# JJanai/slowflow

Measured on AMD Instinct MI355X. Metric: Mpix*solver-iters/s at 1024x436 (whole coarse-to-fine path), higher is better.
Workload: dtype f32

## Files before the change

slowflow_amd/csrc/job.hip:

```cpp
#include <algorithm>
#include <cmath>
#include <cstring>
#include <memory>
#include <vector>

#include "sfa_internal.h"

#pragma clang fp contract(off)

namespace sfa {

enum { P_WX = 0, P_WY, P_UU, P_VV, P_DU, P_DV, P_ODU, P_ODV, P_SH, P_SV, P_A11, P_A12, P_A22, P_B1, P_B2, P_OCC, P_DPSIS, P_COUNT };
struct Level {
    int w = 0, h = 0, pitch = 0, lstride = 0, ref = 0, F = 0, nb = 0;
    bool fused = true;
    long pl = 0, es = 0;
    long off_masks = 0, off_warp = 0, off_stacks = 0, off_tmp = 0;
    float *base = nullptr;
    float *pbase = nullptr;
    float *plane(int i) const { return i < 2 ? pbase + (long)i * pl : base + (long)(i - 2) * pl; }
    float *mask(int s) const { return base + off_masks + (long)s * pl; }
    float *stack(int s, int toref) const { return base + off_stacks + ((long)s * 2 + toref) * 24 * pl; }
    float *warp(int s, int sp1) const { return base + off_warp + (long)(s + sp1) * 3 * pl; }
    float *frame(int f) const { return pbase + 2 * pl + (long)f * 3 * pl; }
    float *tmp() const { return base + off_tmp; }
    Geo geo() const { return Geo{w, h, pitch, pl, es, nb, WMask::first(nb), nullptr}; }
    Geo geo(const WMask &active) const { return Geo{w, h, pitch, pl, es, nb, active, nullptr}; }
    static long persistent_floats(int pitch, int h, int ref) { return (long)pitch * h * (2 + (2L * ref + 1) * 3); }
    static long transient_floats(int pitch, int h, int ref, bool fused) {
        return (long)pitch * h * ((P_COUNT - 2) + 2 * ref + (2L * ref + 1) * 3 + (fused ? 0 : 2L * ref * 2 * 24));
    }
    void layout(float *transient, float *persistent, int w_, int h_, int lstride_, int ref_, int nb_, long es_, bool fused_) {
        base = transient; pbase = persistent; w = w_; h = h_; pitch = dev_pitch(w_); lstride = lstride_; ref = ref_; F = 2 * ref_ + 1; nb = nb_; es = es_; fused = fused_;
        pl = (long)pitch * h;
        off_masks = (long)(P_COUNT - 2) * pl;
        off_warp = off_masks + 2L * ref * pl;
        off_stacks = off_warp + (2L * ref + 1) * 3 * pl;
        off_tmp = off_warp;
    }
};
struct ChannelWeights { const float *dev = nullptr; long pl = 0, es = 0; int pitch = 0, stride0 = 0; };

static const float *pair_image(const Level &L, int s, int sp1) { return (s + sp1 - L.ref == 0) ? L.frame(s + sp1) : L.warp(s, sp1); }

static bool get_derivatives(sfa_ctx *c, const Level &L, const sfa_params &p, const Geo &g, const bool need_toref[2 * SFA_MAX_REF], bool with_smoothness = false) {
    const int ref = L.ref;
    WarpJobs J;
    J.n = 0;
    for (int f = p.one_direction ? ref + 1 : 0; f <= 2 * ref; f++) {
        if (f == ref) continue;
        const int s = f < ref ? f : f - 1;
        J.job[J.n++] = WarpJob{L.frame(f) - L.base, L.warp(f < ref ? f : f - 1, f < ref ? 0 : 1) - L.base, L.mask(s) - L.base, f - ref};
    }
    const bool smoothed = with_smoothness && L.fused &&
                          launch_warp_smooth(c, g, J, L.base, L.plane(P_WX), L.plane(P_WY), p.smoothing, L.plane(P_SH), L.plane(P_SV), L.plane(P_DPSIS), p.alpha, pen(p.robust_reg));
    if (!smoothed) launch_warp_jobs(c, g, J, L.base, L.plane(P_WX), L.plane(P_WY));
    for (int s = p.one_direction ? ref : 0; s < 2 * ref; s++) {
        if (L.fused) continue;
        const float *w_s = pair_image(L, s, 0), *w_sp1 = pair_image(L, s, 1);
        launch_deriv_stack(c, g, L.stack(s, 0), w_s, w_sp1, L.es, L.es);
        if (need_toref[s]) {
            if (s < ref) launch_deriv_stack(c, g, L.stack(s, 1), w_s, L.frame(ref), L.es, L.es);
            else         launch_deriv_stack(c, g, L.stack(s, 1), L.frame(ref), w_sp1, L.es, L.es);
        }
    }
    return smoothed;
}

static int optimize_occlusions(sfa_ctx *c, const Level &L, const sfa_params &p, const Geo &g, DevMem &scratch) {
    const int ref = L.ref;
    const size_t n = (size_t)L.nb * L.pl;
    SFA_TRY(scratch.alloc(c, (2 + kCutWorkPlanes) * n * sizeof(float)));
    float *d0 = scratch.f(), *d1 = d0 + n, *work = d1 + n;
    OccArgs oa;
    memset(&oa, 0, sizeof oa);
    oa.nslots = 2 * ref; oa.hd = p.delta / 3.0f; oa.hg = p.gamma / 3.0f; oa.penalty = p.occlusion_penalty;
    oa.color = pen(p.robust_color); oa.grad = pen(p.robust_grad);
    for (int s = 0; s < 2 * ref; s++) {
        const float *i1 = pair_image(L, s, 0), *i2 = pair_image(L, s, 1);
        const float *r1 = s < ref ? i1 : L.frame(ref), *r2 = s < ref ? L.frame(ref) : i2;
        const int idx = std::max(ref - s - 1, s - ref);
        oa.slot[s] = OccSlot{i1 - L.base, i2 - L.base, r1 - L.base, r2 - L.base, L.off_masks + (long)s * L.pl, p.rho[idx], p.omega[idx], s >= ref ? 0 : 1};
    }
    launch_occ_costs(c, g, oa, L.base, d0, d1, L.pl);
    return run_grid_cut(c, g, L.plane(P_OCC), L.es, d0, d1, work, p.occlusion_alpha);
}


static Term data_term(const Level &L, const sfa_params &p, int slot, int is_ref, float weight, float s) {
    const float *i1 = pair_image(L, slot, 0), *i2 = pair_image(L, slot, 1);
    if (is_ref) { if (slot < L.ref) i2 = L.frame(L.ref); else i1 = L.frame(L.ref); }
    return Term{L.off_stacks + ((long)slot * 2 + is_ref) * 24 * L.pl, L.off_masks + (long)slot * L.pl, weight * (p.delta / 3.0f), weight * (p.gamma / 3.0f), s, is_ref,
                i1 - L.base, i2 - L.base, slot < L.ref};
}
static int data_terms(sfa_ctx *c, const Level &L, const sfa_params &p, const ChannelWeights &cw, AssembleArgs &aa, bool need_toref[2 * SFA_MAX_REF]) {
    const int ref = L.ref;
    memset(&aa, 0, sizeof aa);
    for (int s = 0; s < ref; s++) {
        const int a = ref - 1 - s;
        if (!p.one_direction) {
            if (p.rho[a] > 0) aa.t[aa.n++] = data_term(L, p, s, 0, p.rho[a], (float)(s - ref));
            if (p.omega[a] > 0) { aa.t[aa.n++] = data_term(L, p, s, 1, p.omega[a], (float)(s - ref)); need_toref[s] = true; }
        }
        if (p.rho[s] > 0) aa.t[aa.n++] = data_term(L, p, ref + s, 0, p.rho[s], (float)s);
        if (p.omega[s] > 0) { aa.t[aa.n++] = data_term(L, p, ref + s, 1, p.omega[s], (float)(s + 1)); need_toref[ref + s] = true; }
        aa.data_norm += p.rho[s] + p.omega[s];
    }
    for (int t = 0; t < aa.n; t++)
        if (aa.t[t].is_ref && aa.t[t].s == 0) return set_error(c, SFA_ERR_REF_FRAME, "Frame compared to reference frame is the reference frame itself!");
    aa.one_direction = p.one_direction; aa.dt_norm = p.dataterm_norm;
    aa.color = pen(p.robust_color); aa.grad = pen(p.robust_grad);
    aa.chw = cw.dev; aa.chw_pl = cw.pl; aa.chw_es = cw.es; aa.chw_pitch = cw.pitch; aa.chw_stride0 = cw.stride0; aa.lstride = L.lstride;
    aa.accumulate = 0; aa.do_laplacian = 1;
    return SFA_OK;
}

struct LevelPlan {
// ... 584 lines not shown
```

slowflow_amd/csrc/kernels.hip:

```cpp
#include "sfa_device.h"
#include "sor_device.h"

#pragma clang fp contract(off)

namespace sfa {

__device__ __forceinline__ float psi_vec(const PenaltyDev &p, float xsq) {
    const float e2 = p.eps * p.eps;
    switch (p.id) {
    case 0: return 1.0f;
    case 2: return __fdiv_rn(1.0f, 2.0f * e2 + xsq);
    case 3: {
        float out = __fdiv_rn(1.0f, 2.0f * sqrt_rn(xsq + e2));
        if (sqrt_rn(xsq) > p.trunc) out = 0.0f;
        return out;
    }
    case 4: {
        float t = e2 + xsq;
        t = t * t;
        return __fdiv_rn(e2 + 2.0f * xsq, t);
    }
    default: return __fdiv_rn(1.0f, 2.0f * sqrt_rn(xsq + e2));
    }
}
// ... 11 lines not shown
        t = t * t;
        return (float)((e2d + (double)(2.0f * xsq)) / (double)t);
    }
    default: return (float)(1.0 / (2.0 * __dsqrt_rn((double)xsq + e2d)));
    }
}

__global__ void k_warp(float *__restrict__ dst3, float *__restrict__ mask, const float *__restrict__ src3, const float *__restrict__ wx,
                       const float *__restrict__ wy, Geo g, int factor, long src_es) {
    const int b = blockIdx.z;
    if (!elem_active(g, b)) return;
    const int x = blockIdx.x * BX + threadIdx.x, y = blockIdx.y * BY + threadIdx.y;
    if (x >= g.w || y >= g.h) return;
    dst3 += b * g.es; wx += b * g.es; wy += b * g.es; src3 += b * src_es;
    const size_t o = (size_t)y * g.pitch + x;
    if (factor == 0) {
        for (int k = 0; k < 3; k++) dst3[k * g.pl + o] = src3[k * g.pl + o];
        return;
    }
    const float xx = x + factor * wx[o];
    const float yy = y + factor * wy[o];
    const int xi = floor_to_int_x86(xx), yi = floor_to_int_x86(yy);
    const float dx = xx - xi, dy = yy - yi;
    if (mask) mask[b * g.es + o] = (xx >= 0 && xx <= g.w - 1 && yy >= 0 && yy <= g.h - 1) ? 1.0f : 0.0f;
    const int x1 = clampi(xi, 0, g.w - 1), x2 = clampi(xi + 1, 0, g.w - 1);
    const int y1 = clampi(yi, 0, g.h - 1), y2 = clampi(yi + 1, 0, g.h - 1);
    const float ax = 1.0f - dx, ay = 1.0f - dy;
    for (int k = 0; k < 3; k++) {
        const float *s = src3 + k * g.pl;
        dst3[k * g.pl + o] = s[(size_t)y1 * g.pitch + x1] * ax * ay + s[(size_t)y1 * g.pitch + x2] * dx * ay
                           + s[(size_t)y2 * g.pitch + x1] * ax * dy + s[(size_t)y2 * g.pitch + x2] * dx * dy;
    }
}
template <bool ALLJ>
__global__ void k_warp_jobs(WarpJobs J, float *__restrict__ base, const float *__restrict__ wx, const float *__restrict__ wy, Geo g) {
    const int b = ALLJ ? blockIdx.z : blockIdx.z / J.n, j0 = ALLJ ? 0 : blockIdx.z % J.n;
    if (!elem_active(g, b)) return;
    const int x = blockIdx.x * BX + threadIdx.x, y = blockIdx.y * BY + threadIdx.y;
    if (x >= g.w || y >= g.h) return;
    const long eb = b * g.es;
    const size_t o = (size_t)y * g.pitch + x;
    const float fx0 = wx[eb + o], fy0 = wy[eb + o];
    for (int j = j0; j <= (ALLJ ? J.n - 1 : j0); j++) {
        const int factor = J.job[j].factor;
        const float *src3 = base + eb + J.job[j].src_off;
        float *dst3 = base + eb + J.job[j].dst_off;
        const float xx = x + factor * fx0;
        const float yy = y + factor * fy0;
        const int xi = floor_to_int_x86(xx), yi = floor_to_int_x86(yy);
        const float dx = xx - xi, dy = yy - yi;
        if (J.job[j].mask_off >= 0) base[eb + J.job[j].mask_off + o] = (xx >= 0 && xx <= g.w - 1 && yy >= 0 && yy <= g.h - 1) ? 1.0f : 0.0f;
        const int x1 = clampi(xi, 0, g.w - 1), x2 = clampi(xi + 1, 0, g.w - 1);
        const int y1 = clampi(yi, 0, g.h - 1), y2 = clampi(yi + 1, 0, g.h - 1);
        const float ax = 1.0f - dx, ay = 1.0f - dy;
        float out[3];
#pragma unroll
        for (int k = 0; k < 3; k++) {
            const float *s = src3 + k * g.pl;
            out[k] = s[(size_t)y1 * g.pitch + x1] * ax * ay + s[(size_t)y1 * g.pitch + x2] * dx * ay
                   + s[(size_t)y2 * g.pitch + x1] * ax * dy + s[(size_t)y2 * g.pitch + x2] * dx * dy;
        }
#pragma unroll
        for (int k = 0; k < 3; k++) dst3[k * g.pl + o] = out[k];
    }
}
void launch_warp_jobs(sfa_ctx *c, const Geo &g, const WarpJobs &J, float *base, const float *wx, const float *wy) {
    if (J.n <= 0) return;
    const bool allj = sw_int(Switches::WARP_ALLJ, 1) != 0;
    if (allj) hipLaunchKernelGGL(k_warp_jobs<true>, grid2d(g), block2d(), 0, c->stream, J, base, wx, wy, g);
    else hipLaunchKernelGGL(k_warp_jobs<false>, grid2d(g, J.n), block2d(), 0, c->stream, J, base, wx, wy, g);
}
void launch_warp(sfa_ctx *c, const Geo &g, float *dst3, float *mask, const float *src3, const float *wx, const float *wy, int factor, long src_es) {
    hipLaunchKernelGGL(k_warp, grid2d(g), block2d(), 0, c->stream, dst3, mask, src3, wx, wy, g, factor, src_es);
}


constexpr int DT_X = 64, DT_Y = 16, DT_H = 4, DT_W = DT_X + 2 * DT_H, DT_R = DT_Y + 2 * DT_H;
struct TileAcc {
    const float *t; int x0, y0;
    __device__ __forceinline__ float operator()(int x, int y) const { return t[(y - y0) * DT_W + (x - x0)]; }
};
__global__ void __launch_bounds__(256) k_deriv_stack(float *__restrict__ out24, const float *__restrict__ I1, const float *__restrict__ I2, Geo g, long es1, long es2) {
    __shared__ float sM[DT_R * DT_W], sZ[DT_R * DT_W], sX[DT_R * DT_W], sY[DT_R * DT_W];
    const int b = blockIdx.z / 3, ch = blockIdx.z % 3;
    if (!elem_active(g, b)) return;
    const int x0 = blockIdx.x * DT_X - DT_H, y0 = blockIdx.y * DT_Y - DT_H;
    const float *a = I1 + b * es1 + ch * g.pl, *bb = I2 + b * es2 + ch * g.pl;
    for (int i = threadIdx.x; i < DT_R * DT_W; i += 256) {
        const int x = x0 + i % DT_W, y = y0 + i / DT_W;
        if (x >= 0 && x < g.w && y >= 0 && y < g.h) {
            const size_t o = (size_t)y * g.pitch + x;
            const float va = a[o], vb = bb[o];
            sM[i] = 0.5f * (vb + va);
            sZ[i] = va - vb;
        }
    }
    __syncthreads();
    const TileAcc m{sM, x0, y0};
    constexpr int W1 = DT_X + 4, R1 = DT_Y + 4;
    for (int i = threadIdx.x; i < R1 * W1; i += 256) {
        const int lx = 2 + i % W1, ly = 2 + i / W1;
        const int x = x0 + lx, y = y0 + ly;
        if (x >= 0 && x < g.w && y >= 0 && y < g.h) {
// ... 280 lines not shown
#endif
    auto ld = [](const float *ubase, unsigned boff) { return *reinterpret_cast<const float *>(reinterpret_cast<const char *>(ubase) + boff); };
    auto st = [](float *ubase, unsigned boff, float v) {
        if (SFA_X_WS & 32) __builtin_nontemporal_store(v, reinterpret_cast<float *>(reinterpret_cast<char *>(ubase) + boff));
        else *reinterpret_cast<float *>(reinterpret_cast<char *>(ubase) + boff) = v;
    };
    const unsigned pitch4 = 4u * (unsigned)g.pitch;
    const float *pu = uu_ + eb, *pv = vv_ + eb, *pd = dps_ + eb;
    for (int i = tid; i < SM_R * SM_W; i += 64 * WS_ROWS) {
        const int gx = x0 + i % SM_W, gy = y0 + i / SM_W;
        if (gx >= 0 && gx < g.w && gy >= 0 && gy < g.h) {
            const unsigned o4 = (unsigned)gy * pitch4 + 4u * (unsigned)gx;
            tU[i] = ld(pu, o4); tV[i] = ld(pv, o4); tD[i] = ld(pd, o4);
        }
    }
    __syncthreads();
    const SmTile uu{tU, x0, y0}, vv{tV, x0, y0}, dps{tD, x0, y0};
    const int w = g.w, h = g.h;
    const int x = x0 + 1 + threadIdx.x;
    sh += eb; sv += eb;
    for (int k = 0; k < SM_Y / WS_ROWS; k++) {
        const int y = y0 + 1 + threadIdx.y + WS_ROWS * k;
        if (x >= g.pitch || y >= h) continue;
        const unsigned o4 = (unsigned)y * pitch4 + 4u * (unsigned)x;
        if (x >= w) { st(sh, o4, 0.0f); st(sv, o4, 0.0f); continue; }
        const float fx0 = uu(x, y), fy0 = vv(x, y);
        auto gather = [&](int j, float(&out)[3]) {
            const int factor = J.job[j].factor;
            const float *src3 = base + eb + J.job[j].src_off;
            const float xx = x + factor * fx0;
            const float yy = y + factor * fy0;
            const int xi = floor_to_int_x86(xx), yi = floor_to_int_x86(yy);
            const float dx = xx - xi, dy = yy - yi;
            if (J.job[j].mask_off >= 0) st(base + eb + J.job[j].mask_off, o4, (xx >= 0 && xx <= g.w - 1 && yy >= 0 && yy <= g.h - 1) ? 1.0f : 0.0f);
            const int x1 = clampi(xi, 0, g.w - 1), x2 = clampi(xi + 1, 0, g.w - 1);
            const int y1 = clampi(yi, 0, g.h - 1), y2 = clampi(yi + 1, 0, g.h - 1);
            const float ax = 1.0f - dx, ay = 1.0f - dy;
            const unsigned r1 = (unsigned)y1 * pitch4, r2 = (unsigned)y2 * pitch4, c1 = 4u * (unsigned)x1, c2 = 4u * (unsigned)x2;
            const unsigned o11 = (SFA_X_WS & 1) ? o4 : r1 + c1, o12 = (SFA_X_WS & 1) ? o4 : r1 + c2, o21 = (SFA_X_WS & 1) ? o4 : r2 + c1, o22 = (SFA_X_WS & 1) ? o4 : r2 + c2;
#pragma unroll
            for (int ch = 0; ch < 3; ch++) {
                const float *sp = src3 + ch * g.pl;
                if (SFA_X_WS & 8) { out[ch] = ax * ay + dx * dy; continue; }
#if defined(SFA_WS_LDNT) && SFA_WS_LDNT
                auto ldn = [](const float *ubase, unsigned boff) { return __builtin_nontemporal_load(reinterpret_cast<const float *>(reinterpret_cast<const char *>(ubase) + boff)); };
                out[ch] = ldn(sp, o11) * ax * ay + ldn(sp, o12) * dx * ay + ldn(sp, o21) * ax * dy + ldn(sp, o22) * dx * dy;
#else
                out[ch] = ld(sp, o11) * ax * ay + ld(sp, o12) * dx * ay + ld(sp, o21) * ax * dy + ld(sp, o22) * dx * dy;
#endif
            }
        };
        auto put = [&](int j, const float(&out)[3]) {
            float *dst3 = base + eb + J.job[j].dst_off;
#pragma unroll
            for (int ch = 0; ch < 3; ch++) {
                if (SFA_X_WS & 4) continue;
                if (SFA_WS_NT) __builtin_nontemporal_store(out[ch], reinterpret_cast<float *>(reinterpret_cast<char *>(dst3 + ch * g.pl) + o4));
                else st(dst3 + ch * g.pl, o4, out[ch]);
            }
        };
        float out0[3] = {0, 0, 0}, out1[3] = {0, 0, 0};
        gather(0, out0);
        if (J.n > 1) gather(1, out1);
        float outh = 0.0f, outv = 0.0f;
        if (x < w - 1) {
            const float ux1 = uu(x + 1, y) - uu(x, y), vx1 = vv(x + 1, y) - vv(x, y);
            float t = 0.0f, t2 = 0.0f;
// ... 2 lines not shown
                t2 = 0.5f * (d3y(vv, x, y, h) + d3y(vv, x + 1, y, h));
            }
            t = ux1 * ux1 + t * t;
            t2 = vx1 * vx1 + t2 * t2;
            t = t + t2;
            outh = (dps(x, y) + dps(x + 1, y)) * alpha * ((SFA_X_WS & 2) ? t : psi_scalar(reg, t));
        }
        if (y < h - 1) {
            const float uy1 = uu(x, y + 1) - uu(x, y), vy1 = vv(x, y + 1) - vv(x, y);
            float t = 0.0f, t2 = 0.0f;
            if (method == 1) {
                t = 0.5f * (d3x(uu, x, y, w) + d3x(uu, x, y + 1, w));
                t2 = 0.5f * (d3x(vv, x, y, w) + d3x(vv, x, y + 1, w));
            }
            t = uy1 * uy1 + t * t;
            t2 = vy1 * vy1 + t2 * t2;
            t = t + t2;
            outv = (dps(x, y) + dps(x, y + 1)) * alpha * ((SFA_X_WS & 2) ? t : psi_scalar(reg, t));
        }
        st(sh, o4, outh);
        st(sv, o4, outv);
        put(0, out0);
        if (J.n > 1) put(1, out1);
        for (int j = 2; j < J.n; j++) {
            float o3[3];
            gather(j, o3);
            put(j, o3);
        }
    }
}
bool launch_warp_smooth(sfa_ctx *c, const Geo &g, const WarpJobs &J, float *base, const float *wx, const float *wy, int method, float *sh, float *sv,
                        const float *dpsis, float alpha, PenaltyDev reg) {
    const bool off = sw_given(Switches::NO_WARP_SMOOTH);
    if (off || method > 1 || J.n <= 0) return false;
    if ((unsigned long long)g.pl * 4ull >= (1ull << 32)) return false;
#if defined(SFA_WS_XCD) && SFA_WS_XCD
    const unsigned tiles = (unsigned)((g.pitch + SM_X - 1) / SM_X) * (unsigned)((g.h + SM_Y - 1) / SM_Y) * (unsigned)g.nb;
    hipLaunchKernelGGL(k_warp_smooth, dim3((tiles + 7) / 8 * 8), dim3(64, WS_ROWS), 0, c->stream, J, base, method, sh, sv, wx, wy, dpsis, g, alpha, reg);
#else
    hipLaunchKernelGGL(k_warp_smooth, dim3((g.pitch + SM_X - 1) / SM_X, (g.h + SM_Y - 1) / SM_Y, g.nb), dim3(64, WS_ROWS), 0, c->stream, J, base, method, sh, sv, wx, wy,
                       dpsis, g, alpha, reg);
#endif
    return true;
}

template <class SrcAcc>
__device__ __forceinline__ float laplacian_gather(float bval, const SrcAcc &src, const SrcAcc &wh, const SrcAcc &wv, int x, int y, int w, int h) {
    const float c = src(x, y);
    if (x > 0) bval -= wh(x - 1, y) * (c - src(x - 1, y));
    if (x < w - 1) bval += wh(x, y) * (src(x + 1, y) - c);
    if (y > 0) bval -= wv(x, y - 1) * (c - src(x, y - 1));
    if (y < h - 1) bval += wv(x, y) * (src(x, y + 1) - c);
    return bval;
}
__global__ void k_sub_laplacian(float *__restrict__ dst, const float *__restrict__ src, const float *__restrict__ wh, const float *__restrict__ wv, Geo g) {
    const int b = blockIdx.z;
    const int x = blockIdx.x * BX + threadIdx.x, y = blockIdx.y * BY + threadIdx.y;
    if (x >= g.w || y >= g.h) return;
    PlaneAcc s{src + b * g.es, g.pitch}, h_{wh + b * g.es, g.pitch}, v_{wv + b * g.es, g.pitch};
    const size_t o = b * g.es + (size_t)y * g.pitch + x;
    dst[o] = laplacian_gather(dst[o], s, h_, v_, x, y, g.w, g.h);
}
void launch_sub_laplacian(sfa_ctx *c, const Geo &g, float *dst, const float *src, const float *wh, const float *wv) {
    hipLaunchKernelGGL(k_sub_laplacian, grid2d(g), block2d(), 0, c->stream, dst, src, wh, wv, g);
}

#define EPS2F (0.001f * 0.001f)
// ... 838 lines not shown
    const int dt_norm = FAST ? 1 : a.dt_norm;
    PenaltyDev pcolor = a.color, pgrad = a.grad;
    if (FAST) { pcolor.id = FAST; pgrad.id = FAST; }
    Acc A[NP];
    float u[NP], v[NP], wk[NP][3], fwd[NP], bwd[NP], oc[NP];
    bool ok[NP];
#pragma unroll
    for (int k = 0; k < NP; k++) {
        const int y = y0 + DT_H + ty + NR * k;
        ok[k] = x < g.w && y < g.h;
        A[k].a11 = A[k].a12 = A[k].a22 = A[k].b1 = A[k].b2 = 0.0f;
        u[k] = v[k] = 0.0f; fwd[k] = bwd[k] = 0.0f; oc[k] = 0.0f;
        wk[k][0] = wk[k][1] = wk[k][2] = 1.0f;
        if (!ok[k]) continue;
        const size_t o = (size_t)y * g.pitch + x;
        if (!ZUV) { u[k] = du[eb + o]; v[k] = dv[eb + o]; }
        if (!FAST && a.chw) channel_weights(a, b, x, y, wk[k]);
        if (!(SFA_X_AI & 128)) oc[k] = occ[eb + o];
    }
    const bool need_g = a.do_laplacian || a.op.sa;
    auto stage_epilogue_operands = [&]() {
        if (!need_g) return;
        for (int i0 = 0; i0 < K::NGQ; i0 += NT) {
            const int item = i0 + (int)threadIdx.x;
            const int q = item % K::QM, row = (item / K::QM) % K::GR, pl = item / (K::QM * K::GR);
            const int gy = y0 + DT_H - 1 + row, gx = x0 + 4 * q;
            const float *src = pl == 0 ? uu : pl == 1 ? vv : pl == 2 ? sh : sv;
            if (!(SFA_X_AI & 32) && item < K::NGQ && gy >= 0 && gy < g.h && gx >= 0 && gx + 3 < g.pitch && (pl >= 2 || a.do_laplacian))
                dma16(src + eb + (size_t)gy * g.pitch + gx, lds_addr(lds + 4 * (i0 + 64 * ty)));
        }
    };
    AT_MARK(13);
    if (a.n == 0) stage_epilogue_operands();
    float mk[NP];
    for (int t = 0; t < a.n; t++) {
        const Term &T = a.t[t];
        AT_MARK(0);
        if (t > 0) __syncthreads();
        AT_MARK(1);
        SFA_PRIO(SFA_PRIO_STAGE);
        asm_issue_image_dma<K>(base + eb + T.i1_off, base + eb + T.i2_off, g, x0, y0, tx, ty);
#pragma unroll
        for (int k = 0; k < NP; k++) {
            const size_t o = (size_t)(y0 + DT_H + ty + NR * k) * g.pitch + x;
            mk[k] = ok[k] && !(SFA_X_AI & 128) ? base[eb + T.mask_off + o] : 0.0f;
        }
        AT_MARK(2);
        asm volatile("s_waitcnt vmcnt(0)" ::: "memory");
#pragma unroll
        for (int k = 0; k < NP; k++) {
            asm volatile("" : "+v"(mk[k]), "+v"(oc[k]));
            if (!FAST) asm volatile("" : "+v"(wk[k][0]), "+v"(wk[k][1]), "+v"(wk[k][2]));
            if (!ZUV) asm volatile("" : "+v"(u[k]), "+v"(v[k]));
        }
        AT_MARK(3);
        __syncthreads();
        AT_MARK(4);
        if (t == 0) {
#pragma unroll
            for (int k = 0; k < NP; k++) mask_weights(oc[k], a.data_norm, fwd[k], bwd[k]);
        }
        if (tile_in) asm_convert<K, true>(base + eb + T.i1_off, base + eb + T.i2_off, g, x0, y0);
        else asm_convert<K, false>(base + eb + T.i1_off, base + eb + T.i2_off, g, x0, y0);
        AT_MARK(5);
        AT_MARK(0);
        __syncthreads();
        AT_MARK(6);
        SFA_PRIO(SFA_PRIO_STAGE);
        if (tile_in) asm_stage1<K, true>(g, x0, y0);
        else asm_stage1<K, false>(g, x0, y0);
        AT_MARK(7);
        __syncthreads();
        AT_MARK(8);
        SFA_PRIO(0);
        if (t == a.n - 1) stage_epilogue_operands();
#pragma unroll
        for (int k = 0; k < NP; k++) {
            const int yl = ty + NR * k, y = y0 + DT_H + yl;
            if (y >= g.h) break;
            Px p = asm_pixel_derivatives<K>(g, x0, y0, tx, yl, y);
#pragma unroll
            for (int ch = 0; ch < 3; ch++) p.wk[ch] = FAST ? 1.0f : wk[k][ch];
            if (!ok[k]) continue;
            float m = mk[k];
            if (!a.one_direction || !T.backward) m = T.backward ? 1.0f * bwd[k] * m : 1.0f * fwd[k] * m;
            if (SFA_X_AI & 16) {
                for (int ch = 0; ch < 3; ch++) {
                    A[k].a11 += p.ix[ch] + p.ixx[ch] + m; A[k].a12 += p.iy[ch] + p.ixy[ch]; A[k].a22 += p.iz[ch] + p.iyy[ch]; A[k].b1 += p.ixz[ch]; A[k].b2 += p.iyz[ch];
                }
            } else if (T.is_ref) term_ref<ZUV, FAST != 0>(A[k], p, m, u[k], v[k], T.hd, T.hg, T.s, dt_norm, pcolor, pgrad, a.chain_ok != 0);
            else          term_succ<ZUV, FAST != 0>(A[k], p, m, u[k], v[k], T.hd, T.hg, T.s, dt_norm, pcolor, pgrad, a.chain_ok != 0);
        }
    }
    AT_MARK(0);
    if (need_g) {
        asm volatile("s_waitcnt vmcnt(0)" ::: "memory");
        __syncthreads();
    }
    AT_MARK(9);
    SFA_PRIO(SFA_PRIO_STAGE);
#pragma unroll
    for (int k = 0; k < NP; k++) {
        if (!ok[k]) continue;
        const int yl = ty + NR * k, y = y0 + DT_H + yl;
        asm_epilogue_pixel<K>(a, g, A[k], u[k], v[k], x0, y0, tx, yl, x, y);
        if (!a.op.sa) {
            const size_t o = eb + (size_t)y * g.pitch + x;
            a11[o] = A[k].a11; a12[o] = A[k].a12; a22[o] = A[k].a22; b1[o] = A[k].b1; b2[o] = A[k].b2;
        }
    }
    if (!a.op.sa) return;
    AT_MARK(10);
    __syncthreads();
    AT_MARK(11);
    asm_store_operand_tile<K>(a.op, g, b, x0 + DT_H, y0 + DT_H);
#ifdef SFA_ASM_TIMING
    AT_MARK(12);
// ... 788 lines not shown
```

slowflow_amd/csrc/occlusion.hip:

```cpp
#include "sfa_device.h"
#include <vector>

#include <cstdlib>
#include <utility>

#pragma clang fp contract(off)

namespace sfa {

__device__ __forceinline__ float psi_apply_vec(const PenaltyDev &p, float xsq) {
    const float e2 = p.eps * p.eps;
    switch (p.id) {
    case 0: return xsq;
    case 2: return (float)log(1 + 0.5 * (double)xsq / (double)e2);
    case 3: {
        float out = sqrt_rn(xsq + e2);
        if (sqrt_rn(xsq) > p.trunc) out = sqrt_rn(p.trunc + e2);
        return out;
    }
    case 4: return __fdiv_rn(xsq, (xsq + 1.0f) * (xsq + 1.0f));
    default: return sqrt_rn(xsq + e2);
    }
}

#define DT_SCALE_GRAPHC 0.01f

constexpr int OC_X = 64, OC_Y = 8, OC_W = OC_X + 4, OC_R = OC_Y + 4, OC_NT = 512;
struct OccTileAcc {
    const float *t; int x0, y0;
    __device__ __forceinline__ float operator()(int x, int y) const { return t[(y - y0) * OC_W + (x - x0)]; }
};

__global__ void __launch_bounds__(OC_NT) k_occ_costs(OccArgs a, const float *__restrict__ base, float *__restrict__ d0, float *__restrict__ d1, long des, Geo g) {
    __shared__ float sZ[3][OC_R * OC_W];
    const int b = blockIdx.z;
    if (!elem_active(g, b)) return;
    const long eb = b * g.es;
    const int x0 = blockIdx.x * OC_X - 2, y0 = blockIdx.y * OC_Y - 2;
    const int tx = threadIdx.x & 63;
    const int ty = __builtin_amdgcn_readfirstlane(threadIdx.x >> 6);
    const int x = x0 + 2 + tx, y = y0 + 2 + ty;
    const bool ok = x < g.w && y < g.h;
    const bool y_in = y >= 2 && y + 2 < g.h;
    const int c = (ty + 2) * OC_W + (tx + 2);
    float e[2] = {0.0f, 0.0f}, n[2] = {0.0f, 0.0f};
    for (int s = 0; s < a.nslots; s++) {
        const OccSlot &S = a.slot[s];
        const float m = ok ? base[eb + S.mask_off + (size_t)y * g.pitch + x] : 0.0f;
        float term = 0.0f;
        for (int kind = 0; kind < 2; kind++) {
            const float wgt = kind ? S.omega : S.rho;
            if (wgt == 0.0f && kind == 1) continue;
            const float *pa = base + eb + (kind ? S.r1_off : S.s1_off), *pb = base + eb + (kind ? S.r2_off : S.s2_off);
            __syncthreads();
            constexpr int OC_Q = (OC_W + 2 + 3) / 4;
            for (int i = threadIdx.x; i < 3 * OC_R * OC_Q; i += OC_NT) {
                const int ch = i / (OC_R * OC_Q), r = (i / OC_Q) % OC_R, qa = i % OC_Q;
                const int gy = y0 + r, gx = x0 - 2 + 4 * qa;
                if (gy < 0 || gy >= g.h) continue;
                const size_t ro = ch * g.pl + (size_t)gy * g.pitch;
                float z[4];
                if (gx >= 0 && gx + 3 < g.w) {
                    const float4 va = *reinterpret_cast<const float4 *>(pa + ro + gx), vb = *reinterpret_cast<const float4 *>(pb + ro + gx);
                    z[0] = va.x - vb.x; z[1] = va.y - vb.y; z[2] = va.z - vb.z; z[3] = va.w - vb.w;
                } else {
#pragma unroll
                    for (int e = 0; e < 4; e++) { const int cx = clampi(gx + e, 0, g.w - 1); z[e] = pa[ro + cx] - pb[ro + cx]; }
                }
#pragma unroll
                for (int e = 0; e < 4; e++) {
                    const int q = 4 * qa - 2 + e;
                    if (q >= 0 && q < OC_W) sZ[ch][r * OC_W + q] = z[e];
                }
            }
            __syncthreads();
            if (!ok) continue;
            float iz[3], ixz[3], iyz[3];
#pragma unroll
            for (int ch = 0; ch < 3; ch++) {
                const float *Z = sZ[ch];
                iz[ch] = Z[c];
                ixz[ch] = tap5(Z[c - 2], Z[c - 1], Z[c], Z[c + 1], Z[c + 2]);
                if (y_in) iyz[ch] = tap5(Z[c - 2 * OC_W], Z[c - OC_W], Z[c], Z[c + OC_W], Z[c + 2 * OC_W]);
                else      iyz[ch] = d5y(OccTileAcc{Z, x0, y0}, x, y, g.h);
            }
            const float pc = psi_apply_vec(a.color, iz[0] * iz[0] + iz[1] * iz[1] + iz[2] * iz[2]);
            const float pg = psi_apply_vec(a.grad, ixz[0] * ixz[0] + ixz[1] * ixz[1] + ixz[2] * ixz[2] + iyz[0] * iyz[0] + iyz[1] * iyz[1] + iyz[2] * iyz[2]);
            if (kind == 0) term = wgt * a.hd * m * pc;
            else           term += wgt * a.hd * m * pc;
            term += wgt * a.hg * m * pg;
        }
        const int l = S.label;
        e[l] += term;
        n[l] += m * (S.rho + S.rho + S.omega + S.omega);
    }
    if (!ok) return;
    const size_t o = b * des + (size_t)y * g.pitch + x;
#pragma unroll
    for (int l = 0; l < 2; l++) {
        if (n[l] == 0) n[l] = 1;
        const float cst = __fdiv_rn(DT_SCALE_GRAPHC * e[l], n[l]) + a.penalty * l;
        (l ? d1 : d0)[o] = cst;
    }
}
void launch_occ_costs(sfa_ctx *c, const Geo &g, const OccArgs &a, const float *base, float *d0, float *d1, long des) {
    hipLaunchKernelGGL(k_occ_costs, dim3((g.w + OC_X - 1) / OC_X, (g.h + OC_Y - 1) / OC_Y, g.nb), dim3(OC_NT), 0, c->stream, a, base, d0, d1, des, g);
}

constexpr int kCutInf = 1 << 30;
struct CutPlanes { float *e, *tc, *c[4], *f[4]; int *hgt, *hgt_next; };
__device__ __forceinline__ void cut_raise(unsigned *flag) {
    if (!__hip_atomic_load(flag, __ATOMIC_RELAXED, __HIP_MEMORY_SCOPE_AGENT)) atomicOr(flag, 1u);
}
struct CutTiles { int *idle, *idle_next, *dirty, *dirty_next; };
__device__ __forceinline__ int cut_tile(int b) { return (b * gridDim.y + blockIdx.y) * gridDim.x + blockIdx.x; }
template <class Pred>
__device__ __forceinline__ bool cut_tile_nb_any(const int *flag, int t, Pred pred) {
    return (blockIdx.x > 0 && pred(flag[t - 1])) || (blockIdx.x + 1 < gridDim.x && pred(flag[t + 1])) ||
           (blockIdx.y > 0 && pred(flag[t - (int)gridDim.x])) || (blockIdx.y + 1 < gridDim.y && pred(flag[t + (int)gridDim.x]));
}
__device__ __forceinline__ long cut_nb(int d, int x, int y, int w, int h, int pitch) {
    switch (d) {
    case 0: return x + 1 < w ? 1 : 0;
    case 1: return x > 0 ? -1 : 0;
    case 2: return y + 1 < h ? pitch : 0;
    default: return y > 0 ? -pitch : 0;
    }
}

constexpr int kCountRows = 8;
__global__ void __launch_bounds__(BX *BY) k_cut_count(const float *__restrict__ d0, const float *__restrict__ d1, unsigned *__restrict__ counts, Geo g) {
    __shared__ unsigned s_cnt[2];
    const int b = blockIdx.z;
    const int x = blockIdx.x * BX + threadIdx.x;
    if (threadIdx.x == 0 && threadIdx.y == 0) { s_cnt[0] = 0; s_cnt[1] = 0; }
    __syncthreads();
    unsigned pos = 0, neg = 0;
    if (x < g.w)
        for (int y = blockIdx.y * BY + threadIdx.y; y < g.h; y += gridDim.y * BY) {
// ... 576 lines not shown
```

slowflow_amd/csrc/sfa_device.h:

```cpp
#pragma once
#include "sfa_internal.h"

#pragma clang fp contract(off)

namespace sfa {

#define BX 64
#define BY 4

static inline dim3 grid2d(const Geo &g, int zmul = 1) { return dim3((g.w + BX - 1) / BX, (g.h + BY - 1) / BY, g.nb * zmul); }
static inline dim3 block2d() { return dim3(BX, BY, 1); }

__device__ __forceinline__ bool elem_active(const WMask &active, const unsigned long long *amask, int b) {
    const unsigned long long m = amask ? (active.w[b >> 6] & amask[b >> 6]) : active.w[b >> 6];
    return (m >> (b & 63)) & 1ull;
}
__device__ __forceinline__ bool elem_active(const Geo &g, int b) { return elem_active(g.active, g.amask, b); }
__device__ __forceinline__ int clampi(int a, int lo, int hi) { return a < lo ? lo : (a > hi ? hi : a); }
__device__ __forceinline__ int floor_to_int_x86(float v) {
    const float f = floorf(v);
    return (f >= -2147483648.0f && f < 2147483648.0f) ? (int)f : (-2147483647 - 1);
}

#define C5_0 (1.0f / 12.0f)
#define C5_1 (-8.0f / 12.0f)
#define C5_2 (-0.0f)
#define C5_3 (8.0f / 12.0f)
#define C5_4 (-(1.0f / 12.0f))
#define C3_0 (-0.5f)
#define C3_1 (-0.0f)
#define C3_2 (0.5f)

__device__ __forceinline__ float tap5(float m2, float m1, float c, float p1, float p2) {
#if defined(SFA_X_NO_CENTRE_TAP)
    return C5_0 * m2 + C5_1 * m1 + C5_3 * p1 + C5_4 * p2;
#else
    return C5_0 * m2 + C5_1 * m1 + C5_2 * c + C5_3 * p1 + C5_4 * p2;
#endif
}

template <class F>
__device__ __forceinline__ float d5x(F f, int x, int y, int w) {
    return tap5(f(clampi(x - 2, 0, w - 1), y), f(clampi(x - 1, 0, w - 1), y), f(x, y), f(clampi(x + 1, 0, w - 1), y), f(clampi(x + 2, 0, w - 1), y));
}
template <class F>
__device__ __forceinline__ float d5y(F f, int x, int y, int h) {
    if (y == 0) return (C5_0 + C5_1 + C5_2) * f(x, 0) + C5_3 * f(x, 1) + C5_4 * f(x, 2);
    if (y == 1) return (C5_0 + C5_1) * f(x, 0) + C5_2 * f(x, 1) + C5_3 * f(x, 2) + C5_4 * f(x, 3);
    if (y == h - 2) return C5_0 * f(x, y - 2) + C5_1 * f(x, y - 1) + C5_2 * f(x, y) + (C5_3 + C5_4) * f(x, y + 1);
    if (y == h - 1) return C5_0 * f(x, y - 2) + C5_1 * f(x, y - 1) + (C5_2 + C5_3 + C5_4) * f(x, y);
    return tap5(f(x, y - 2), f(x, y - 1), f(x, y), f(x, y + 1), f(x, y + 2));
}
template <class F>
__device__ __forceinline__ float d3x(F f, int x, int y, int w) {
// ... 31 lines not shown
```

slowflow_amd/csrc/sfa_internal.h:

```cpp
#pragma once
#include <hip/hip_runtime.h>

#include <cstdarg>
#include <cstdio>
#include <string>
#include <vector>

#include "../../include/slowflow_amd.h"
#include "dev_view.h"

#pragma clang fp contract(off)

namespace sfa {

constexpr int kMaskWords = 2;
constexpr int kMaxBatch = 64 * kMaskWords;
struct WMask {
    unsigned long long w[kMaskWords];
    __host__ __device__ bool test(int b) const { return (w[b >> 6] >> (b & 63)) & 1ull; }
    __host__ __device__ void clear(int b) { w[b >> 6] &= ~(1ull << (b & 63)); }
    __host__ __device__ void set(int b) { w[b >> 6] |= 1ull << (b & 63); }
    __host__ __device__ bool any() const { unsigned long long o = 0; for (int i = 0; i < kMaskWords; i++) o |= w[i]; return o != 0; }
    __host__ __device__ bool operator==(const WMask &o) const { bool e = true; for (int i = 0; i < kMaskWords; i++) e = e && w[i] == o.w[i]; return e; }
    __host__ __device__ bool operator!=(const WMask &o) const { return !(*this == o); }
// ... 148 lines not shown
    int penalty;
    double eps_sq;
    float weight;
};
struct EnergyPlan { AdaptTab tab; EnergyArgs a; int rJ, J, w, h, gw, gh, incr, start, r, NN; size_t lds; };
int energy_plan(sfa_ctx *ctx, const sfa_energy_params *p, int r_Jets, int Jets, int w, int h, EnergyPlan *out);
void energy_records_device(sfa_ctx *ctx, size_t nf, int w, int h, const float *frames, float *der, void *rec);
struct EnergyWork { double *U, *V; unsigned long long *occ; float *jc, *oc; double *ep; };
int energies_device(sfa_ctx *ctx, const EnergyPlan &pl, int n, const double *acc_u, const double *acc_v, const int *tracked, const void *rec, bool identity,
                    const void *fwd, const void *bwd, const EnergyWork &wk, double *energy, unsigned long long *occ_out, size_t out_seg, double *adapted_u,
                    double *adapted_v, size_t adapted_seg);
int energies_adapted_device(sfa_ctx *ctx, const EnergyPlan &pl, int n, const int *tracked, const EnergyWork &wk, double *adapted_u, double *adapted_v, size_t adapted_seg);
struct FuseWork {
    const double *U, *V, *energy; const unsigned long long *occ; const float *weight;
    unsigned char *nl, *lab; double *theta, *P, *M; unsigned char *xcur, *xbest;
    int *slot; double *fu, *fv; unsigned char *out_occ; double *seg_energy, *seg_bound; int *seg_iters;
};
int fuse_device(sfa_ctx *ctx, const sfa_fuse_params *p, int n, int K, int Jets, int w, int h, int gw, int gh, const FuseWork &f, hipEvent_t *ev);

int consistent_regions_device(sfa_ctx *ctx, int n, int w, int h, const int *tracked, const int *full, int min_size, int *T, int *P, int *S, unsigned char *mask,
                              int *kept);
size_t fill_matches_blocks(int nx, int ny);
int fill_matches_device(sfa_ctx *ctx, int n, int J, int w, int h, const double *acc_u, const double *acc_v, const unsigned char *mask, const int *xs, int nx,
                        const int *ys, int ny, int divisor, int *block_count, float *matches, int *count);
int fill_trajectories_device(sfa_ctx *ctx, int n, int J, int w, int h, int stride, const float *flow_x, const float *flow_y, int scale, double *acc_u,
                             double *acc_v, int *tracked);

struct Geo { int w, h, pitch; long pl; long es; int nb; WMask active; const unsigned long long *amask; };

struct PenaltyDev { int id; float eps, trunc; };
inline PenaltyDev pen(const sfa_penalty &p) { return PenaltyDev{p.id, p.eps, p.trunc}; }

struct WarpJob { long src_off, dst_off, mask_off; int factor; };
struct WarpJobs { WarpJob job[4 * SFA_MAX_REF]; int n; };
void launch_warp_jobs(sfa_ctx *c, const Geo &g, const WarpJobs &J, float *base, const float *wx, const float *wy);
bool launch_warp_smooth(sfa_ctx *c, const Geo &g, const WarpJobs &J, float *base, const float *wx, const float *wy, int method, float *sh, float *sv,
                        const float *dpsis, float alpha, PenaltyDev reg);
void launch_warp(sfa_ctx *c, const Geo &g, float *dst3, float *mask, const float *src3, const float *wx, const float *wy, int factor,
                 long src_es );
void launch_deriv_stack(sfa_ctx *c, const Geo &g, float *out24, const float *I1, const float *I2, long es1, long es2);
void launch_convolve(sfa_ctx *c, const Geo &g, float *dst, const float *src, int order, int horiz, int nplanes);
void launch_dpsis(sfa_ctx *c, const Geo &g, float *dst, const float *im3, long im_es, float coef, const float avg[3], const float stdv[3], int hbit);
void launch_smoothness(sfa_ctx *c, const Geo &g, int method, float *sh, float *sv, const float *uu, const float *vv, const float *dpsis,
                       float alpha, PenaltyDev reg);
void launch_sub_laplacian(sfa_ctx *c, const Geo &g, float *dst, const float *src, const float *wh, const float *wv);
void launch_mask_weight(sfa_ctx *c, const Geo &g, float *masks, const float *occ, float data_norm, int ref, int one_direction);
void launch_fill(sfa_ctx *c, float *p, size_t n, float v);
void launch_division_chain(sfa_ctx *c, const float *a, const float *b, float *q_chain, float *q_exact, unsigned char *admitted, size_t n);
void launch_fill_planes(sfa_ctx *c, const Geo &g, float *p, int nplanes, float v);
void launch_zero_planes(sfa_ctx *c, const Geo &g, float *p, int nplanes);
void launch_outer_threshold(sfa_ctx *c, const Geo &g, const double *red, float thres, const float *dfa = nullptr, const float *dfb = nullptr);
void launch_set_mask(sfa_ctx *c, const WMask &v);

struct SorOperandOut {
    float4 *sa = nullptr, *sb = nullptr; unsigned long long *x = nullptr; unsigned *flags = nullptr;
    long ent = 0; int RP = 0, G = 0, ntasks = 0, nb = 0;
};
struct Term {
    long stack_off; long mask_off; float hd, hg, s; int is_ref;
    long i1_off, i2_off; int backward;
};
struct AssembleArgs {
    Term t[kMaxTerms];
    int n;
    int dt_norm;
    PenaltyDev color, grad;
    const float *chw; long chw_pl; long chw_es; int chw_pitch; int chw_stride0; int lstride;
    int accumulate;
    int do_laplacian;
    float data_norm; int one_direction;
    SorOperandOut op;
    int zero_duv;
    int chain_ok = 0;
};
void launch_assemble(sfa_ctx *c, const Geo &g, const AssembleArgs &a, const float *base , float *a11, float *a12,
                     float *a22, float *b1, float *b2, const float *du, const float *dv, const float *uu, const float *vv, const float *sh, const float *sv);

int launch_assemble_images(sfa_ctx *c, const Geo &g, const AssembleArgs &a, const float *base, float *a11, float *a12, float *a22, float *b1, float *b2,
                            const float *du, const float *dv, const float *uu, const float *vv, const float *sh, const float *sv, const float *occ);

void launch_smoothness_2f(sfa_ctx *c, const Geo &g, float *sh, float *sv, const float *uu, const float *vv, const float *dpsis, float half_alpha);
void launch_data_2f(sfa_ctx *c, const Geo &g, const float *D, const float *mask, const float *du, const float *dv, float *a11, float *a12, float *a22, float *b1,
                    float *b2, const float *wx, const float *wy, const float *sh, const float *sv, float hd, float hg);
void launch_data_2f_fused(sfa_ctx *c, const Geo &g, const float *I1, const float *I2, const float *mask, const float *du, const float *dv, float *a11, float *a12,
                          float *a22, float *b1, float *b2, const float *wx, const float *wy, const float *sh, const float *sv, float hd, float hg);

struct OccSlot {
    long s1_off, s2_off;
    long r1_off, r2_off;
    long mask_off;
    float rho, omega;
    int label;
};
struct OccArgs { OccSlot slot[2 * SFA_MAX_REF]; int nslots; float hd, hg, penalty; PenaltyDev color, grad; };
void launch_occ_costs(sfa_ctx *c, const Geo &g, const OccArgs &a, const float *base, float *d0, float *d1, long d_es );
constexpr int kCutWorkPlanes = 13;
int run_grid_cut(sfa_ctx *c, const Geo &g, float *occ, long occ_es, const float *d0, const float *d1, float *work, float alpha);

void launch_update_inner(sfa_ctx *c, const Geo &g, float *uu, float *vv, const float *wx, const float *wy, const float *du, const float *dv,
                         const float *old_du, const float *old_dv, double *red , float *dfa = nullptr, float *dfb = nullptr);
void launch_update_inner_x(sfa_ctx *c, const Geo &g, float *uu, float *vv, const float *wx, const float *wy, const SorOperandOut &x, const float *old_du,
                           const float *old_dv, float *du_out, float *dv_out, double *red, float *dfa = nullptr, float *dfb = nullptr);
void launch_exact_norms(sfa_ctx *c, const Geo &g, const float *dfa, const float *dfb, const WMask &which, float *out);
void launch_update_outer_x(sfa_ctx *c, const Geo &g, float *uu, float *vv, float *wx, float *wy, const SorOperandOut &x, double *red, float *dfa = nullptr,
                           float *dfb = nullptr);
void launch_update_outer(sfa_ctx *c, const Geo &g, float *wx, float *wy, const float *uu, const float *vv, double *red, float *dfa = nullptr, float *dfb = nullptr);
void launch_copy_planes(sfa_ctx *c, const Geo &g, float *dst, const float *src, int nplanes, long dst_es, long src_es);
void launch_scale_plane(sfa_ctx *c, const Geo &g, float *p, float s);

constexpr int kMaxBlurRadius = 16, kMaxBlurTaps = 2 * kMaxBlurRadius + 1;
int launch_gauss_blur(sfa_ctx *c, const Geo &g, float *dst, float *tmp, const float *src, int nplanes, const float *taps, int radius);
void launch_resize(sfa_ctx *c, float *dst, int dw, int dh, int dpitch, long dpl, long des, const float *src, int sw, int sh, int spitch, long spl, long ses,
                   int nplanes, int nb, float post_scale);
void launch_resize_flow(sfa_ctx *c, float *dstx, float *dsty, int dw, int dh, int dpitch, long des, const float *srcx, const float *srcy, int sw, int sh, int spitch,
                        long ses, int nb, float post_x, float post_y);
void launch_resize_scaled(sfa_ctx *c, float *dst, int dw, int dh, int dpitch, long dpl, long des, const float *src, int sw, int sh, int spitch, long spl,
                          long ses, int nplanes, int nb, float post_scale, double scale_x, double scale_y);
struct PyrInfo { int fused, td, lds; };
bool launch_pyr_down(sfa_ctx *c, float *dst, int dw, int dh, int dpitch, long dpl, long des, const float *src, int sw, int sh, int spitch, long spl, long ses,
                     int nplanes, int nb, const float *taps, int radius, PyrInfo *info = nullptr);
int pyramid_step(sfa_ctx *c, float *dst, int dw, int dh, int dpitch, long dpl, long des, const float *src, int sw, int sh, int spitch, long spl, long ses, int nplanes,
                 int nb, const float *taps, int radius, float *tmp, PyrInfo *info = nullptr);
void launch_presmooth(sfa_ctx *c, const Geo &g, float *dst, float *tmp, const float *src, int nplanes, float sigma);
void launch_normalize_sums(sfa_ctx *c, const Geo &g, const float *frames3, double *red );
void launch_normalize_apply(sfa_ctx *c, const Geo &g, float *frames3, const double avg[3], const double stdv[3]);
__attribute__((visibility("hidden"))) int cv_gauss_taps(float sigma, float k[kMaxBlurTaps]);

struct PackSrc { const void *p; int dtype; long long sw, sf, sc, sr, sx; };
// ... 69 lines not shown
```

Measured before the change: 255,800.

## Pack warp in-bounds masks into 64-bit ballot words

Warp kernels now write the in-bounds mask as one 64-bit ballot word per wave instead of one float per pixel. The assemble and occlusion-cost kernels read that word through a scalar constant-address load and extract the lane's bit with v_cndmask. This shrinks mask write and read traffic by a large factor and moves mask loads to the scalar path. It relies on BX==64, pitch aligned to 64, and wave64 lanes mapping to consecutive x, and it applies only on the fused path.

```diff
diff --git a/slowflow_amd/csrc/job.hip b/slowflow_amd/csrc/job.hip
--- a/slowflow_amd/csrc/job.hip
+++ b/slowflow_amd/csrc/job.hip
@@ -1,5 +1,7 @@
 #include <algorithm>
+#include <cassert>
 #include <cmath>
+#include <cstdint>
 #include <cstring>
 #include <memory>
 #include <vector>
@@ -47,6 +49,8 @@
     const int ref = L.ref;
     WarpJobs J;
     J.n = 0;
+    J.mask_bits = L.fused ? 1 : 0;
+    for (int s = 0; s < 2 * ref; s++) assert(L.pitch % 64 == 0 && reinterpret_cast<uintptr_t>(L.mask(s)) % 8 == 0 && (L.es * sizeof(float)) % 8 == 0);
     for (int f = p.one_direction ? ref + 1 : 0; f <= 2 * ref; f++) {
         if (f == ref) continue;
         const int s = f < ref ? f : f - 1;
@@ -82,7 +86,7 @@
         const int idx = std::max(ref - s - 1, s - ref);
         oa.slot[s] = OccSlot{i1 - L.base, i2 - L.base, r1 - L.base, r2 - L.base, L.off_masks + (long)s * L.pl, p.rho[idx], p.omega[idx], s >= ref ? 0 : 1};
     }
-    launch_occ_costs(c, g, oa, L.base, d0, d1, L.pl);
+    launch_occ_costs(c, g, oa, L.base, d0, d1, L.pl, L.fused);
     return run_grid_cut(c, g, L.plane(P_OCC), L.es, d0, d1, work, p.occlusion_alpha);
 }
 
diff --git a/slowflow_amd/csrc/kernels.hip b/slowflow_amd/csrc/kernels.hip
--- a/slowflow_amd/csrc/kernels.hip
+++ b/slowflow_amd/csrc/kernels.hip
@@ -67,8 +67,9 @@
                            + s[(size_t)y2 * g.pitch + x1] * ax * dy + s[(size_t)y2 * g.pitch + x2] * dx * dy;
     }
 }
-template <bool ALLJ>
+template <bool ALLJ, bool BITS>
 __global__ void k_warp_jobs(WarpJobs J, float *__restrict__ base, const float *__restrict__ wx, const float *__restrict__ wy, Geo g) {
+    static_assert(BX == 64, "one mask word per wave");
     const int b = ALLJ ? blockIdx.z : blockIdx.z / J.n, j0 = ALLJ ? 0 : blockIdx.z % J.n;
     if (!elem_active(g, b)) return;
     const int x = blockIdx.x * BX + threadIdx.x, y = blockIdx.y * BY + threadIdx.y;
@@ -84,7 +85,13 @@
         const float yy = y + factor * fy0;
         const int xi = floor_to_int_x86(xx), yi = floor_to_int_x86(yy);
         const float dx = xx - xi, dy = yy - yi;
-        if (J.job[j].mask_off >= 0) base[eb + J.job[j].mask_off + o] = (xx >= 0 && xx <= g.w - 1 && yy >= 0 && yy <= g.h - 1) ? 1.0f : 0.0f;
+        if (J.job[j].mask_off >= 0) {
+            const bool inside = xx >= 0 && xx <= g.w - 1 && yy >= 0 && yy <= g.h - 1;
+            if (BITS) {
+                const unsigned long long word = __ballot(inside);
+                if (threadIdx.x == 0) reinterpret_cast<unsigned long long *>(base + eb + J.job[j].mask_off)[mask_word_index(y, blockIdx.x, g.pitch)] = word;
+            } else base[eb + J.job[j].mask_off + o] = inside ? 1.0f : 0.0f;
+        }
         const int x1 = clampi(xi, 0, g.w - 1), x2 = clampi(xi + 1, 0, g.w - 1);
         const int y1 = clampi(yi, 0, g.h - 1), y2 = clampi(yi + 1, 0, g.h - 1);
         const float ax = 1.0f - dx, ay = 1.0f - dy;
@@ -102,8 +109,9 @@
 void launch_warp_jobs(sfa_ctx *c, const Geo &g, const WarpJobs &J, float *base, const float *wx, const float *wy) {
     if (J.n <= 0) return;
     const bool allj = sw_int(Switches::WARP_ALLJ, 1) != 0;
-    if (allj) hipLaunchKernelGGL(k_warp_jobs<true>, grid2d(g), block2d(), 0, c->stream, J, base, wx, wy, g);
-    else hipLaunchKernelGGL(k_warp_jobs<false>, grid2d(g, J.n), block2d(), 0, c->stream, J, base, wx, wy, g);
+    const bool bits = J.mask_bits != 0;
+    if (allj) hipLaunchKernelGGL((bits ? k_warp_jobs<true, true> : k_warp_jobs<true, false>), grid2d(g), block2d(), 0, c->stream, J, base, wx, wy, g);
+    else hipLaunchKernelGGL((bits ? k_warp_jobs<false, true> : k_warp_jobs<false, false>), grid2d(g, J.n), block2d(), 0, c->stream, J, base, wx, wy, g);
 }
 void launch_warp(sfa_ctx *c, const Geo &g, float *dst3, float *mask, const float *src3, const float *wx, const float *wy, int factor, long src_es) {
     hipLaunchKernelGGL(k_warp, grid2d(g), block2d(), 0, c->stream, dst3, mask, src3, wx, wy, g, factor, src_es);
@@ -450,7 +458,10 @@
             const float yy = y + factor * fy0;
             const int xi = floor_to_int_x86(xx), yi = floor_to_int_x86(yy);
             const float dx = xx - xi, dy = yy - yi;
-            if (J.job[j].mask_off >= 0) st(base + eb + J.job[j].mask_off, o4, (xx >= 0 && xx <= g.w - 1 && yy >= 0 && yy <= g.h - 1) ? 1.0f : 0.0f);
+            if (J.job[j].mask_off >= 0) {
+                const unsigned long long word = __ballot(xx >= 0 && xx <= g.w - 1 && yy >= 0 && yy <= g.h - 1);
+                if (threadIdx.x == 0) reinterpret_cast<unsigned long long *>(base + eb + J.job[j].mask_off)[mask_word_index(y, x >> 6, g.pitch)] = word;
+            }
             const int x1 = clampi(xi, 0, g.w - 1), x2 = clampi(xi + 1, 0, g.w - 1);
             const int y1 = clampi(yi, 0, g.h - 1), y2 = clampi(yi + 1, 0, g.h - 1);
             const float ax = 1.0f - dx, ay = 1.0f - dy;
@@ -519,7 +530,7 @@
 bool launch_warp_smooth(sfa_ctx *c, const Geo &g, const WarpJobs &J, float *base, const float *wx, const float *wy, int method, float *sh, float *sv,
                         const float *dpsis, float alpha, PenaltyDev reg) {
     const bool off = sw_given(Switches::NO_WARP_SMOOTH);
-    if (off || method > 1 || J.n <= 0) return false;
+    if (off || method > 1 || J.n <= 0 || !J.mask_bits) return false;
     if ((unsigned long long)g.pl * 4ull >= (1ull << 32)) return false;
 #if defined(SFA_WS_XCD) && SFA_WS_XCD
     const unsigned tiles = (unsigned)((g.pitch + SM_X - 1) / SM_X) * (unsigned)((g.h + SM_Y - 1) / SM_Y) * (unsigned)g.nb;
@@ -1424,7 +1435,7 @@
     };
     AT_MARK(13);
     if (a.n == 0) stage_epilogue_operands();
-    float mk[NP];
+    unsigned long long mw[NP];
     for (int t = 0; t < a.n; t++) {
         const Term &T = a.t[t];
         AT_MARK(0);
@@ -1434,14 +1445,14 @@
         asm_issue_image_dma<K>(base + eb + T.i1_off, base + eb + T.i2_off, g, x0, y0, tx, ty);
 #pragma unroll
         for (int k = 0; k < NP; k++) {
-            const size_t o = (size_t)(y0 + DT_H + ty + NR * k) * g.pitch + x;
-            mk[k] = ok[k] && !(SFA_X_AI & 128) ? base[eb + T.mask_off + o] : 0.0f;
+            const int y = y0 + DT_H + ty + NR * k;
+            mw[k] = y < g.h && !(SFA_X_AI & 128) ? mask_word(base + eb + T.mask_off, mask_word_index(y, bx, g.pitch)) : 0ull;
         }
         AT_MARK(2);
         asm volatile("s_waitcnt vmcnt(0)" ::: "memory");
 #pragma unroll
         for (int k = 0; k < NP; k++) {
-            asm volatile("" : "+v"(mk[k]), "+v"(oc[k]));
+            asm volatile("" : "+v"(oc[k]));
             if (!FAST) asm volatile("" : "+v"(wk[k][0]), "+v"(wk[k][1]), "+v"(wk[k][2]));
             if (!ZUV) asm volatile("" : "+v"(u[k]), "+v"(v[k]));
         }
@@ -1474,7 +1485,7 @@
 #pragma unroll
             for (int ch = 0; ch < 3; ch++) p.wk[ch] = FAST ? 1.0f : wk[k][ch];
             if (!ok[k]) continue;
-            float m = mk[k];
+            float m = mask_lane_bit(mw[k]);
             if (!a.one_direction || !T.backward) m = T.backward ? 1.0f * bwd[k] * m : 1.0f * fwd[k] * m;
             if (SFA_X_AI & 16) {
                 for (int ch = 0; ch < 3; ch++) {
diff --git a/slowflow_amd/csrc/occlusion.hip b/slowflow_amd/csrc/occlusion.hip
--- a/slowflow_amd/csrc/occlusion.hip
+++ b/slowflow_amd/csrc/occlusion.hip
@@ -31,6 +31,7 @@
     __device__ __forceinline__ float operator()(int x, int y) const { return t[(y - y0) * OC_W + (x - x0)]; }
 };
 
+template <bool BITS>
 __global__ void __launch_bounds__(OC_NT) k_occ_costs(OccArgs a, const float *__restrict__ base, float *__restrict__ d0, float *__restrict__ d1, long des, Geo g) {
     __shared__ float sZ[3][OC_R * OC_W];
     const int b = blockIdx.z;
@@ -46,7 +47,11 @@
     float e[2] = {0.0f, 0.0f}, n[2] = {0.0f, 0.0f};
     for (int s = 0; s < a.nslots; s++) {
         const OccSlot &S = a.slot[s];
-        const float m = ok ? base[eb + S.mask_off + (size_t)y * g.pitch + x] : 0.0f;
+        float m = 0.0f;
+        if (BITS) {
+            const unsigned long long word = y < g.h ? mask_word(base + eb + S.mask_off, mask_word_index(y, blockIdx.x, g.pitch)) : 0ull;
+            m = mask_lane_bit(word);
+        } else if (ok) m = base[eb + S.mask_off + (size_t)y * g.pitch + x];
         float term = 0.0f;
         for (int kind = 0; kind < 2; kind++) {
             const float wgt = kind ? S.omega : S.rho;
@@ -103,8 +108,8 @@
         (l ? d1 : d0)[o] = cst;
     }
 }
-void launch_occ_costs(sfa_ctx *c, const Geo &g, const OccArgs &a, const float *base, float *d0, float *d1, long des) {
-    hipLaunchKernelGGL(k_occ_costs, dim3((g.w + OC_X - 1) / OC_X, (g.h + OC_Y - 1) / OC_Y, g.nb), dim3(OC_NT), 0, c->stream, a, base, d0, d1, des, g);
+void launch_occ_costs(sfa_ctx *c, const Geo &g, const OccArgs &a, const float *base, float *d0, float *d1, long des, bool mask_bits) {
+    hipLaunchKernelGGL(mask_bits ? k_occ_costs<true> : k_occ_costs<false>, dim3((g.w + OC_X - 1) / OC_X, (g.h + OC_Y - 1) / OC_Y, g.nb), dim3(OC_NT), 0, c->stream, a, base, d0, d1, des, g);
 }
 
 constexpr int kCutInf = 1 << 30;
diff --git a/slowflow_amd/csrc/sfa_device.h b/slowflow_amd/csrc/sfa_device.h
--- a/slowflow_amd/csrc/sfa_device.h
+++ b/slowflow_amd/csrc/sfa_device.h
@@ -20,6 +20,17 @@
 __device__ __forceinline__ int floor_to_int_x86(float v) {
     const float f = floorf(v);
     return (f >= -2147483648.0f && f < 2147483648.0f) ? (int)f : (-2147483647 - 1);
+}
+
+__device__ __forceinline__ size_t mask_word_index(int y, int cx, int pitch) { return (size_t)y * (size_t)(pitch >> 6) + (size_t)cx; }
+__device__ __forceinline__ unsigned long long mask_word(const float *region, size_t index) {
+    typedef const unsigned long long __attribute__((address_space(4))) *const_words;
+    return *(const_words)(reinterpret_cast<const unsigned long long *>(region) + index);
+}
+__device__ __forceinline__ float mask_lane_bit(unsigned long long word) {
+    float m;
+    asm("v_cndmask_b32_e64 %0, 0, 1.0, %1" : "=v"(m) : "s"(word));
+    return m;
 }
 
 #define C5_0 (1.0f / 12.0f)
diff --git a/slowflow_amd/csrc/sfa_internal.h b/slowflow_amd/csrc/sfa_internal.h
--- a/slowflow_amd/csrc/sfa_internal.h
+++ b/slowflow_amd/csrc/sfa_internal.h
@@ -204,7 +204,7 @@
 inline PenaltyDev pen(const sfa_penalty &p) { return PenaltyDev{p.id, p.eps, p.trunc}; }
 
 struct WarpJob { long src_off, dst_off, mask_off; int factor; };
-struct WarpJobs { WarpJob job[4 * SFA_MAX_REF]; int n; };
+struct WarpJobs { WarpJob job[4 * SFA_MAX_REF]; int n; int mask_bits; };
 void launch_warp_jobs(sfa_ctx *c, const Geo &g, const WarpJobs &J, float *base, const float *wx, const float *wy);
 bool launch_warp_smooth(sfa_ctx *c, const Geo &g, const WarpJobs &J, float *base, const float *wx, const float *wy, int method, float *sh, float *sv,
                         const float *dpsis, float alpha, PenaltyDev reg);
@@ -265,7 +265,8 @@
     int label;
 };
 struct OccArgs { OccSlot slot[2 * SFA_MAX_REF]; int nslots; float hd, hg, penalty; PenaltyDev color, grad; };
-void launch_occ_costs(sfa_ctx *c, const Geo &g, const OccArgs &a, const float *base, float *d0, float *d1, long d_es );
+void launch_occ_costs(sfa_ctx *c, const Geo &g, const OccArgs &a, const float *base, float *d0, float *d1, long d_es ,
+                      bool mask_bits = false);
 constexpr int kCutWorkPlanes = 13;
 int run_grid_cut(sfa_ctx *c, const Geo &g, float *occ, long occ_es, const float *d0, const float *d1, float *work, float alpha);
 
```

Result: faster. 258,400 (median of 6 runs) (+1.0%).
